# dfdazac/grapes

Measured on AMD Instinct MI355X. Metric: sampled edges aggregated/sec, ogbn-products 3-layer GFlowNet, higher is better.
Workload: dtype f32

## Files before the change

grapes_amd/_lib.py:

```python
from __future__ import annotations

import ctypes as C
import os

_HERE = os.path.dirname(os.path.abspath(__file__))
DIAG_LIB_PATH = os.path.join(_HERE, "libgrapes_hip_diag.so")
DIAG = os.environ.get("GRAPES_DIAG", "0") == "1"
LIB_PATH = os.environ.get("GRAPES_LIB_PATH") or (DIAG_LIB_PATH if DIAG else os.path.join(_HERE, "libgrapes_hip.so"))
ABI_MAJOR, ABI_MINOR = 3, 2


def diag_switch(name: str, default: str) -> str:
    if os.environ.get("GRAPES_DIAG", "0") == "1":
        return os.environ.get(name, default)
    return default


P = C.c_void_p
I32 = C.c_int32
I64 = C.c_int64
U32 = C.c_uint32
U64 = C.c_uint64
F32 = C.c_float
SZ = C.c_size_t
# ... 135 lines not shown
    "grapes_sampler_head_bwd_multi_phase": (I32, [I32, P, P, P, P, P, P, P, P, P, P, P, P, I32, P, P, P, I32, P]),
    "grapes_linear_bias_act_head_fwd_strided": (I32, [P, I32, P, P, I32, P, P, P, I32, P, I32, I32, P]),
    "grapes_linear_bwd_weight_gated_strided": (I32, [P, P, I32, P, I32, P, P, P, P, P, I32, I32, I32, P, P]),
    "grapes_linear_bwd_weight_gated_workspace_bytes": (SZ, [I32, I32, I32]),
    "grapes_linear_bwd_weight_gated": (I32, [P, P, P, P, P, I32, P, I32, I32, I32, P, P, P, P, P]),
    "grapes_linear_bwd_weight_gated_multi": (I32, [I32, P, P, P, P, P, P, P, P, P, I32, I32, I32, P, P]),
    "grapes_linear_bwd_weight_slabs_bytes": (SZ, [I32, I32, I32]),
    "grapes_linear_bwd_weight_slabs": (I32, [P, P, P, I32, P, I32, I32, I32, P, P]),
    "grapes_linear_bwd_weight_slabs_and_input": (I32, [P, P, P, P, P, I32, P, I32, I32, I32, P, P]),
    "grapes_slab_reduce_sets": (I32, [I32, P, P, P, I32, P, I32, P]),
    "grapes_gcn_aggregate_narrow_pair": (I32, [P, P, P, P, P, P, P, P, P, I32, P, P]),
    "grapes_linear_relu_head_fwd_bits": (I32, [P, I32, P, P, P, P, P, I32, P, I32, I32, P]),
    "grapes_linear_relu_head_fwd_bits_pair": (I32, [P, I32, P, P, P, P, P, P, I32, P, P, P, P, P, I32, I32, P, I32, I32, P]),
    "grapes_linear_bwd_weight_bits_multi_cols": (I32, [I32, P, P, P, P, P, P, P, P, P, P, I32, P, P, I32, I32, I32, P, P]),
    "grapes_linear_bwd_weight_bits_pair_cols": (I32, [I32, P, P, P, P, P, P, P, P, P, P, I32, P, P, I32, P, P, P, P, P, P, I32, I32, I32, P, P]),
    "grapes_gcn_aggregate_gather_fwd": (I32, [P, I32, I32, P, P, U32, P, I32, P, P, P, P, P, I32, P, P]),
    "grapes_gcn_aggregate_gather_fwd_peers": (I32, [P, P, I32, I32, I32, P, P, U32, P, I32, P, P, P, P, P, I32, P, P]),
    "grapes_peer_export": (I32, [P, P, P]),
    "grapes_peer_open": (I32, [P, U64, P]),
    "grapes_peer_close": (I32, [P, U64]),
    "grapes_peer_copy": (I32, [P, P, SZ, P]),
    "grapes_gcn_aggregate_workspace_bytes": (SZ, [I32, I32]),
    "grapes_gcn_aggregate_fwd": (I32, [P, P, P, P, P, P, I32, P, I32, I32, P, P, I32, P, P]),
    "grapes_gcn_aggregate_fwd_head": (I32, [P, P, P, P, P, P, I32, P, I32, I32, P, P, P, P]),
    "grapes_gcn_aggregate_fwd_prescaled": (I32, [P, P, P, P, P, P, I32, P, I32, I32, P, P, I32, P, P]),
    "grapes_scale_rows": (I32, [P, P, P, I64, I32, P]),
    "grapes_gcn_aggregate_bwd_rank1_workspace_bytes": (SZ, [I32, I32]),
    "grapes_gcn_aggregate_bwd_rank1": (I32, [P, P, P, P, P, P, P, P, P, I32, I32, P, I32, P, P, I32, P, P]),
    "grapes_gcn_aggregate_bwd_rank1_bits": (I32, [P, P, P, P, P, P, P, P, P, P, I32, I32, P, I32, P, P, I32, P, P]),
    "grapes_gcn_aggregate_bwd_rank1_bits_multi": (I32, [I32, P, P, P, P, P, P, P, P, P, P, P, P, P, I32, P, P, P, P, P]),
# ... 104 lines not shown
```

grapes_amd/csrc/gemm_kernels.hip:

```cpp
#include <type_traits>
#include "common.h"
#include <cstdlib>

typedef float f32x16 __attribute__((ext_vector_type(16)));

#define GB_M 128
#define GB_N 128
#define GB_K 16
#define GB_LD 132

struct GatherOp { const int32_t* ids; const uint32_t* code; const uint32_t* d_epoch; uint32_t epoch; int F; uint32_t mask; };

template <bool KMAJOR, bool VEC>
__device__ __forceinline__ void gemm_load_tile(const float* __restrict__ P, long long ld, int r0, int R, int k0,
                                               int kend, int tid, float4 (&v)[2], const float* __restrict__ G = nullptr,
                                               int ones_at = -1, const float* __restrict__ row_scale = nullptr,
                                               const float* __restrict__ col_vec = nullptr, float4* cs2 = nullptr,
                                               const GatherOp* go = nullptr, bool do_cs2 = false) {
    if (VEC) {
#pragma unroll
        for (int i = 0; i < 2; ++i) {
            int k, r;
            bool ok;
            long long off;
// ... 1805 lines not shown
}

#define DS_NT 128
#ifdef GRAPES_STAMPS
#define DWS_STAMP(slot, T0) do { if (grapes_stamp_ptr && threadIdx.x == (T0) && blockIdx.x < 64) grapes_stamp_ptr[blockIdx.x * 16 + (slot)] = wall_clock64(); } while (0)
#define DWS_STAMP_IT(it_, slot) do { if ((it_) == 6) { DWS_STAMP(slot, 0); DWS_STAMP((slot) + 6, 256); } } while (0)
#else
#define DWS_STAMP(slot, T0) do { } while (0)
#define DWS_STAMP_IT(it_, slot) do { } while (0)
#endif
#define DS_MINROWS 128
__host__ __device__ __forceinline__ int dw_share(int total, int nwg, bool min_rows) {
    const int per = (total + nwg - 1) / nwg;
    return (min_rows && per < DS_MINROWS) ? DS_MINROWS : per;
}
struct DwAlt { int nwg0; int first_seg; int Nin; const float* cv; float* slabs; float* cs_db; };
struct DwsRegs { uint32_t gw[8]; float4 xb[4]; float rsb[4]; float rso; int rows; float4 xb2[4]; float rsb2[4]; float rso2; };
struct DwsCtx { int M, Nin, kb, ac4, bshift, hb, bc4, ok_, hb2, bc42, ok2_, lane; bool a_role, b_role, o_role, b2_role, o2_role; };
__device__ __forceinline__ int dws_sw(int n) { return n ^ ((n >> 3) & 3); }
template <int ROLE, int NT, int G>
__device__ __forceinline__ void dws_stage_slice(const DwsRegs& R, const DwsCtx& c, uint4* __restrict__ WA, char* __restrict__ WB,
                                                uint4* __restrict__ dummy) {
    constexpr int B_PL = 4 * NT;
    char* dm = reinterpret_cast<char*>(&dummy[c.lane]);
    if constexpr (G < 4) {
        constexpr int u = G;
        if constexpr (ROLE == 0) {
            uint32_t e[4];
#pragma unroll
            for (int pq = 0; pq < 4; ++pq) {
                const uint32_t n0 = (8 * c.kb + 2 * pq < R.rows) ? (R.gw[2 * pq] >> c.bshift) & 15u : 0u;
// ... 56 lines not shown
}
template <int ROLE, int NT>
__device__ __forceinline__ void dws_stage_set(const DwsRegs& R, const DwsCtx& c, uint4* __restrict__ WA, char* __restrict__ WB,
                                              uint4* __restrict__ dummy) {
    dws_stage_slice<ROLE, NT, 0>(R, c, WA, WB, dummy);
    dws_stage_slice<ROLE, NT, 1>(R, c, WA, WB, dummy);
    dws_stage_slice<ROLE, NT, 2>(R, c, WA, WB, dummy);
    dws_stage_slice<ROLE, NT, 3>(R, c, WA, WB, dummy);
    dws_stage_slice<ROLE, NT, 4>(R, c, WA, WB, dummy);
}
template <bool BITS, int NT = 128>
__global__ __launch_bounds__(512, 1) void gemm_dw_split_k(DwSegs sg, const float* __restrict__ cv_, int M, int Nin_,
                                                          float* __restrict__ slabs_, float* __restrict__ cs_db_,
                                                          float* __restrict__ cs_head, DwAlt alt) {
    extern __shared__ uint4 ds_smem[];
    const bool dual = alt.nwg0 < (int)gridDim.x, p1 = dual && (int)blockIdx.x >= alt.nwg0;
    const int bid = p1 ? (int)blockIdx.x - alt.nwg0 : (int)blockIdx.x;
    const int nwg = p1 ? (int)gridDim.x - alt.nwg0 : (dual ? alt.nwg0 : (int)gridDim.x);
    const int seg_lo = p1 ? alt.first_seg : 0, seg_hi = (dual && !p1) ? alt.first_seg : sg.nseg;
    const int Nin = p1 ? alt.Nin : Nin_;
    const float* __restrict__ cv = p1 ? alt.cv : cv_;
    float* __restrict__ slabs = p1 ? alt.slabs : slabs_;
    float* __restrict__ cs_db = p1 ? alt.cs_db : cs_db_;
    auto sw = [](int n) { return n ^ ((n >> 3) & 3); };
    constexpr int A_IMG = 4 * DW_MAXM, B_PL = 4 * NT, BUF = A_IMG + 3 * B_PL;
    constexpr int TN = NT / 32;
    const int tid = threadIdx.x, lane = tid & 63, wid = tid >> 6;
    const int li = lane & 31, h = lane >> 5;
    DWS_STAMP(0, 0);
    for (int i = tid; i < 2 * BUF; i += 512) ds_smem[i] = make_uint4(0u, 0u, 0u, 0u);
    int nrows[4], off[5];
    off[0] = 0;
    {
// ... 343 lines not shown
    if (BITS) {
    } else if (cs_head) {
        __syncthreads();
        float* red = reinterpret_cast<float*>(ds_smem);
        if (a_role) *reinterpret_cast<float4*>(&red[kb * M + 4 * ac4]) = cs2;
        __syncthreads();
        if (tid < M) cs_head[(long long)bid * M + tid] = ((red[tid] + red[M + tid]) + red[2 * M + tid]) + red[3 * M + tid];
    }
}
#define SR1_G 8
struct Sr1Prob {
    const float* slabs; const float* tslabs; const float* cv; const float* W1; const float* b1;
    float* dw; float* db; float* dwh; int nwg, Nin, seg_lo, seg_hi;
    int dw_cols;
};
template <int NC, int G>
__global__ __launch_bounds__(NC * G) void slab_reduce_rank1_k(DwSegs sg, Sr1Prob pa, Sr1Prob pb, int M, int accumulate) {
    __shared__ float red[NC / 64];
    const Sr1Prob P = blockIdx.y ? pb : pa;
    const int Nin = P.Nin;
    const int m = blockIdx.x, g = threadIdx.x / NC, n = threadIdx.x - g * NC;
    const bool is_s = n < Nin, is_t = n == Nin;
    int cnt[4];
#pragma unroll
    for (int q = 0; q < 4; ++q) {
        const bool has = q < sg.nseg && sg.d_n[q];
        const int32_t raw = *(has ? sg.d_n[q] : reinterpret_cast<const int32_t*>(P.cv));
        cnt[q] = has ? raw : 0x7fffffff;
    }
    const float c = P.cv[m];
    const float wrow = (g == 0 && P.dwh) ? (is_s ? P.W1[(long long)m * Nin + n] : (is_t ? P.b1[m] : 0.f)) : 0.f;
    float* o = is_s ? (n < P.dw_cols ? P.dw + (long long)m * P.dw_cols + n : nullptr) : ((is_t && P.db) ? P.db + m : nullptr);
    const float prev = (g == 0 && accumulate && o) ? *o : 0.f;
    int total = 0;
#pragma unroll
    for (int q = 0; q < 4; ++q)
        total += (q >= P.seg_lo && q < P.seg_hi) ? (cnt[q] < sg.n_cap[q] ? (cnt[q] > 0 ? cnt[q] : 0) : sg.n_cap[q]) : 0;
    const int per = dw_share(total, P.nwg, true);
    const int live = total > 0 ? (total + per - 1) / per : 0;
    constexpr int Q = NC / 4, NG = NC * G / Q;
    __shared__ float part4[NG][NC];
    const int q4 = threadIdx.x % Q, g4 = threadIdx.x / Q;
    const bool q_s = 4 * q4 < Nin, q_t = 4 * q4 == Nin;
    float4 a4 = make_float4(0.f, 0.f, 0.f, 0.f);
    if (q_s || q_t) {
// ... 5 lines not shown
                const int z = zb + u * NG < live ? zb + u * NG : live - 1;
                v[u] = q_t ? make_float4(P.tslabs[(long long)z * M + m], 0.f, 0.f, 0.f)
                           : *reinterpret_cast<const float4*>(base + (long long)z * Nin);
            }
#pragma unroll
            for (int u = 0; u < 8; ++u)
                if (zb + u * NG < live) { a4.x += v[u].x; a4.y += v[u].y; a4.z += v[u].z; a4.w += v[u].w; }
        }
    }
    if (4 * q4 + 3 < NC) *reinterpret_cast<float4*>(&part4[g4][4 * q4]) = a4;
    __syncthreads();
    if (g == 0) {
        float sum = part4[0][n];
#pragma unroll 8
        for (int q = 1; q < NG; ++q) sum += part4[q][n];
        if (o) *o = prev + c * sum;
        if (P.dwh) {
            const float p = wave_sum(sum * wrow);
            if ((n & 63) == 0) red[n >> 6] = p;
        }
    }
    __syncthreads();
    if (P.dwh && threadIdx.x == 0) {
        float t = red[0] + red[1];
        if (NC > 128) t += red[2];
        P.dwh[m] = accumulate ? P.dwh[m] + t : t;
    }
}

#define DS_NT_WIDE 160
static inline bool dw_split_ok(int f_in, int f_out, bool bits = false) {
    const bool shape = f_out % 32 == 0 && f_out >= 32 && f_out <= DW_MAXM && f_in % 4 == 0 && f_in >= 4;
    if (shape && 8 * (f_in / 4) + DW_KC <= 256) return true;
    return bits && shape && f_in + 1 <= DS_NT_WIDE && 8 * (f_in / 4) + DW_KC <= 256 + 64;
}
static inline bool dw_split_narrow(int f_in) { return 8 * (f_in / 4) + DW_KC <= 256; }

static inline bool dw_rank1_ok(int f_in, int f_out) {
    return f_out % 32 == 0 && f_out >= 32 && f_out <= DW_MAXM && f_in % 4 == 0 && f_in >= 4 && f_in + 1 <= DW_NT &&
           (512 % (f_out / 4)) == 0;
}

static inline bool fused_dw_ok(const float* dout, const float* gate, const float* x, int f_in, int f_out) {
    return grapes_aligned16(dout) && grapes_aligned16(x) && (!gate || grapes_aligned16(gate)) && f_in % 4 == 0 && f_out % 4 == 0 &&
           f_in % GB_N != 0;
}

#define DW_BLOCKS 256
#define DW_BLOCKS_SECOND 32
struct DwSecond { const float* col_vec; const float* w1; const float* b1; float* dw; float* dbias; float* dw_head; int f_in; };
static int launch_dw_rank1(int nseg, const float* const* gate, const float* const* x, const float* const* row_scale,
                           const int32_t* const* d_n, const int32_t* n_cap, const float* col_vec, float* dw, float* dbias,
                           float* dw_head, int f_in, int f_out, int accumulate, void* workspace, hipStream_t s,
                           const int32_t* x_stride = nullptr ,
                           const uint32_t* const* bits = nullptr ,
                           const float* w1 = nullptr, const float* b1 = nullptr,
                           const struct DwSecond* second = nullptr ,
                           int dw_cols = 0 ) {
    static bool attr_set = false;
    const size_t lds = (size_t)(2 * DW_KC * DW_LDA + 2 * DW_KC * DW_LDB) * sizeof(float);
    if (!attr_set) {
        hipError_t e = hipFuncSetAttribute((const void*)gemm_dw_rank1_k, hipFuncAttributeMaxDynamicSharedMemorySize, (int)lds);
        if (e != hipSuccess) return (int)e;
        attr_set = true;
    }
    DwSegs sg;
    sg.nseg = nseg;
    for (int h = 0; h < 4; ++h) {
        const int q = h < nseg ? h : 0;
        sg.gate[h] = gate ? gate[q] : nullptr; sg.x[h] = x[q]; sg.rs[h] = row_scale[q]; sg.d_n[h] = d_n[q]; sg.n_cap[h] = h < nseg ? n_cap[q] : 0;
        sg.ldx[h] = (x_stride && x_stride[q] > 0) ? x_stride[q] : f_in;
        sg.bits[h] = bits ? bits[q] : nullptr;
    }
// ... 20 lines not shown
            hipError_t e = hipFuncSetAttribute((const void*)gemm_dw_split_k<false>, hipFuncAttributeMaxDynamicSharedMemorySize, (int)l128);
            if (e != hipSuccess) return (int)e;
            e = hipFuncSetAttribute((const void*)gemm_dw_split_k<true>, hipFuncAttributeMaxDynamicSharedMemorySize, (int)l128);
            if (e != hipSuccess) return (int)e;
            e = hipFuncSetAttribute((const void*)gemm_dw_split_k<true, DS_NT_WIDE>, hipFuncAttributeMaxDynamicSharedMemorySize, (int)l160);
            if (e != hipSuccess) return (int)e;
            attr2_set = true;
        }
        if (bits) {
            static int second_wgs = -1;
            if (second_wgs < 0) { const char* e = grapes_tune_env("GRAPES_DW_SECOND_WGS"); second_wgs = e ? atoi(e) : DW_BLOCKS_SECOND;
                                  if (second_wgs < 8 || second_wgs > 128) second_wgs = DW_BLOCKS_SECOND; }
            const int nwg0 = second ? DW_BLOCKS - second_wgs : DW_BLOCKS;
            float* w_dw2 = w_dw + (size_t)nwg0 * slab;
            float* w_db2 = w_db + (size_t)nwg0 * f_out;
            const DwAlt alt{nwg0, second ? nseg - 1 : nseg, second ? second->f_in : f_in, second ? second->col_vec : col_vec, w_dw2, w_db2};
            if (wide)
                hipLaunchKernelGGL((gemm_dw_split_k<true, DS_NT_WIDE>), dim3(DW_BLOCKS), dim3(512), lds2, s, sg, col_vec, f_out, f_in, w_dw, w_db,
                                   (float*)nullptr, alt);
            else
                hipLaunchKernelGGL(gemm_dw_split_k<true>, dim3(DW_BLOCKS), dim3(512), lds2, s, sg, col_vec, f_out, f_in, w_dw, w_db,
                                   (float*)nullptr, alt);
            GRAPES_LAUNCH_CHECK();
            const Sr1Prob pa{w_dw, w_db, col_vec, w1, b1, dw, dbias, dw_head, nwg0, f_in, 0, second ? nseg - 1 : nseg,
                             dw_cols > 0 ? dw_cols : f_in};
            const Sr1Prob pb = second ? Sr1Prob{w_dw2, w_db2, second->col_vec, second->w1, second->b1, second->dw, second->dbias,
                                                second->dw_head, DW_BLOCKS - nwg0, second->f_in, nseg - 1, nseg, second->f_in} : pa;
            if (wide)
                hipLaunchKernelGGL((slab_reduce_rank1_k<192, 5>), dim3(f_out, second ? 2 : 1), dim3(192 * 5), 0, s, sg, pa, pb, f_out, accumulate);
            else
                hipLaunchKernelGGL((slab_reduce_rank1_k<128, SR1_G>), dim3(f_out, second ? 2 : 1), dim3(128 * SR1_G), 0, s, sg, pa, pb, f_out, accumulate);
            GRAPES_LAUNCH_CHECK();
            return 0;
        }
        const DwAlt none{DW_BLOCKS, nseg, f_in, col_vec, w_dw, w_db};
        hipLaunchKernelGGL(gemm_dw_split_k<false>, dim3(DW_BLOCKS), dim3(512), lds2, s, sg, col_vec, f_out, f_in, w_dw,
                           dbias ? w_db : nullptr, dw_head ? w_dh : nullptr, none);
    } else {
        hipLaunchKernelGGL(gemm_dw_rank1_k, dim3(DW_BLOCKS), dim3(512), lds, s, sg, col_vec, f_out, f_in, w_dw,
                           dbias ? w_db : nullptr, dw_head ? w_dh : nullptr);
    }
    GRAPES_LAUNCH_CHECK();
    int grid = grapes_div_up(slab, 64); if (grid > 4096) grid = 4096;
    const int g2 = grid + (dbias ? grapes_div_up(f_out, 64) : 0) + (dw_head ? grapes_div_up(f_out, 64) : 0);
    hipLaunchKernelGGL(slab_reduce_k, dim3(g2), dim3(256), 0, s, (const float*)w_dw, dw, slab, DW_BLOCKS, (const int32_t*)nullptr, 1,
                       accumulate, (const float*)(dbias ? w_db : nullptr), dbias, (long long)(dbias ? f_out : 0),
                       (const float*)(dw_head ? w_dh : nullptr), dw_head, (long long)(dw_head ? f_out : 0));
    GRAPES_LAUNCH_CHECK();
    return 0;
}
// ... 265 lines not shown
    if (dw_cols < 0 || dw_cols > f_in || (dw_cols > 0 && f_in - dw_cols > 3)) return GRAPES_EINVAL;
    if (dw_head && (!w1 || !b1)) return GRAPES_EINVAL;
    int nmax = 0;
    for (int h = 0; h < nseg; ++h) {
        if (!gate_bits[h] || !x[h] || !row_scale[h] || n_cap[h] <= 0) return GRAPES_EINVAL;
        if (x_stride && x_stride[h] > 0 && (x_stride[h] < f_in || (x_stride[h] & 3))) return GRAPES_EINVAL;
        if (!grapes_aligned16(x[h])) return GRAPES_EALIGN;
        nmax = n_cap[h] > nmax ? n_cap[h] : nmax;
    }
    if (!grapes_aligned16(col_vec)) return GRAPES_EALIGN;
    if (!grapes_split_gemm_available(nmax > 2048 ? nmax : 2048, f_in, f_out)) return GRAPES_EINVAL;
    if (dw_cols > 0 && dw_cols != f_in && !dw_split_ok(f_in, f_out, true)) return GRAPES_EINVAL;
    return launch_dw_rank1(nseg, nullptr, x, row_scale, d_n, n_cap, col_vec, dw, dbias, dw_head, f_in, f_out, accumulate, workspace,
                           (hipStream_t)stream, x_stride, gate_bits, w1, b1, nullptr, dw_cols);
}
extern "C" int grapes_linear_bwd_weight_bits_pair_cols(int32_t nseg, const uint32_t* const* gate_bits, const float* const* x,
                                                       const int32_t* x_stride, const float* const* row_scale,
                                                       const int32_t* const* d_n, const int32_t* n_cap, const float* col_vec,
                                                       const float* w1, const float* b1, float* dw, int32_t dw_cols, float* dbias,
                                                       float* dw_head, int32_t f_in, const float* col_vec_b, const float* w1_b,
                                                       const float* b1_b, float* dw_b, float* dbias_b, float* dw_head_b,
                                                       int32_t f_in_b, int32_t f_out, int32_t accumulate, void* workspace,
                                                       grapes_stream_t stream) {
    if (nseg < 1 || nseg > 3 || !gate_bits || !x || !row_scale || !d_n || !n_cap || !col_vec || !dw || !workspace) return GRAPES_EINVAL;
    if (dw_cols < 0 || dw_cols > f_in || (dw_cols > 0 && f_in - dw_cols > 3)) return GRAPES_EINVAL;
    if (!col_vec_b || !dw_b || f_in_b <= 0 || f_in_b > f_in) return GRAPES_EINVAL;
    if ((dw_head && (!w1 || !b1)) || (dw_head_b && (!w1_b || !b1_b))) return GRAPES_EINVAL;
    int nmax = 0;
    for (int h = 0; h <= nseg; ++h) {
        const int fi = h < nseg ? f_in : f_in_b;
        if (!gate_bits[h] || !x[h] || !row_scale[h] || n_cap[h] <= 0) return GRAPES_EINVAL;
        if (x_stride && x_stride[h] > 0 && (x_stride[h] < fi || (x_stride[h] & 3))) return GRAPES_EINVAL;
        if (!grapes_aligned16(x[h])) return GRAPES_EALIGN;
        nmax = n_cap[h] > nmax ? n_cap[h] : nmax;
    }
    if (!grapes_aligned16(col_vec) || !grapes_aligned16(col_vec_b)) return GRAPES_EALIGN;
    if (!grapes_split_gemm_available(nmax > 2048 ? nmax : 2048, f_in, f_out) ||
        !grapes_split_gemm_available(nmax > 2048 ? nmax : 2048, f_in_b, f_out)) return GRAPES_EINVAL;
    int32_t strides[4];
    for (int h = 0; h <= nseg; ++h) strides[h] = (x_stride && x_stride[h] > 0) ? x_stride[h] : (h < nseg ? f_in : f_in_b);
    const DwSecond sec{col_vec_b, w1_b, b1_b, dw_b, dbias_b, dw_head_b, f_in_b};
    return launch_dw_rank1(nseg + 1, nullptr, x, row_scale, d_n, n_cap, col_vec, dw, dbias, dw_head, f_in, f_out, accumulate, workspace,
                           (hipStream_t)stream, strides, gate_bits, w1, b1, &sec, dw_cols);
}
```

grapes_amd/ops.py:

```python
from __future__ import annotations

from typing import List, Optional

import ctypes as _C
import os

import torch

from . import _lib
from ._lib import diag_switch as _sw

_i32 = torch.int32
_i64 = torch.int64
_f32 = torch.float32


def lib():
    return _lib.load()


def _stream() -> int:
    try:
        return torch._C._cuda_getCurrentRawStream(torch._C._cuda_getDevice())
    except AttributeError:
# ... 823 lines not shown
        raise ValueError("linear_bwd_weight_bits_multi: w1 must be a dense [f_out, f_in] matrix and b1 [f_out]")
    dw_cols = _dw_cols(dw, fo, fi, "linear_bwd_weight_bits_multi")
    strides = (C.c_int32 * nseg)(*[_row_strided(x, fi, "linear_bwd_weight_bits_multi") for x in xs])
    arr = lambda ts: (C.c_void_p * nseg)(*[t.data_ptr() for t in ts])
    caps = (C.c_int32 * nseg)(*[x.shape[0] for x in xs])
    ws = _ws(lib().grapes_linear_bwd_weight_gated_workspace_bytes(1, fi, fo), dw.device)
    _lib.check(lib().grapes_linear_bwd_weight_bits_multi_cols(nseg, arr([b.words for b in bits]), arr(xs), strides, arr(row_scales),
                                                              arr(d_ns), caps, _p(col_vec), _p(w1), _p(b1), _p(dw), dw_cols,
                                                              _p(dbias), _p(dw_head), fi, fo, 1 if accumulate else 0, _p(ws),
                                                              _stream()),
               "linear_bwd_weight_bits_multi")
    return dw


def linear_bwd_weight_bits_pair(bits, xs, row_scales, d_ns, col_vec, w1, b1, dw, dbias, dw_head,
                                bits_b, x_b, row_scale_b, d_n_b, col_vec_b, w1_b, b1_b, dw_b, dbias_b, dw_head_b, accumulate=False):
    import ctypes as C
    nseg = len(bits)
    if not (1 <= nseg <= 3 and len(xs) == nseg and len(row_scales) == nseg and len(d_ns) == nseg):
        raise ValueError("1..3 row sets of layer a with matching operand lists")
    for t in list(row_scales) + [row_scale_b, col_vec, col_vec_b, dw, dw_b, w1, b1, w1_b, b1_b]:
        _chk(t, _f32, "operand")
    fo, fi, fib = bits[0].f_out, xs[0].shape[1], x_b.shape[1]
    if (bits_b.f_out != fo or tuple(w1.shape) != (fo, fi) or tuple(w1_b.shape) != (fo, fib) or not w1.is_contiguous() or
            not w1_b.is_contiguous()):
        raise ValueError("linear_bwd_weight_bits_pair: dense [f_out, f_in] weights of one f_out")
    allx = list(xs) + [x_b]
    strides = (C.c_int32 * (nseg + 1))(*[_row_strided(x, fi if i < nseg else fib, "linear_bwd_weight_bits_pair") for i, x in enumerate(allx)])
    arr = lambda ts: (C.c_void_p * (nseg + 1))(*[t.data_ptr() for t in ts])
    caps = (C.c_int32 * (nseg + 1))(*[x.shape[0] for x in allx])
    ws = _ws(lib().grapes_linear_bwd_weight_gated_workspace_bytes(1, fi, fo), dw.device)
    dw_cols = _dw_cols(dw, fo, fi, "linear_bwd_weight_bits_pair")
    _lib.check(lib().grapes_linear_bwd_weight_bits_pair_cols(
        nseg, arr([b.words for b in bits] + [bits_b.words]), arr(allx), strides, arr(list(row_scales) + [row_scale_b]),
        arr(list(d_ns) + [d_n_b]), caps, _p(col_vec), _p(w1), _p(b1), _p(dw), dw_cols, _p(dbias), _p(dw_head), fi,
        _p(col_vec_b), _p(w1_b), _p(b1_b), _p(dw_b), _p(dbias_b), _p(dw_head_b), fib, fo, 1 if accumulate else 0, _p(ws),
        _stream()), "linear_bwd_weight_bits_pair")
    return dw, dw_b


def pad_features(X):
    F = X.shape[1]
    if F % 4 == 0:
        return X.contiguous(), F
    Xp = torch.zeros((X.shape[0], (F + 3) // 4 * 4), dtype=X.dtype, device=X.device)
    Xp[:, :F] = X
    return Xp, F


class FeaturePlanes:

    def __init__(self, Xp: torch.Tensor):
        _chk(Xp, _f32, "X")
# ... 1527 lines not shown
```

grapes_amd/step_graph.py:

```python
from __future__ import annotations

import contextlib
import copy
from typing import Dict, List, Optional

import os

import torch

from ._lib import diag_switch as _sw
import torch.nn as nn

from . import ops
from .capture import SegmentedGraph
from .graph import DeviceGraph


class _FirstLayer:

    def __init__(self, conv, F, num_ind, legacy=False):
        self.conv, self.F, self.num_ind = conv, F, num_ind
        self.K = F + num_ind
        self.Kp = self.K if legacy else (self.K + 3) // 4 * 4
        self.agg_first = legacy or self.K < conv.out_channels or conv.out_channels % 4 != 0
# ... 789 lines not shown
            main_s.wait_stream(self._side)
        elif not cb_done:
            self._classifier_backward(s)

    def _nets_backward(self, s, carry_bwd) -> bool:
        hops, num_ind, ep = self.hops, self.num_ind, self.epoch_t
        gf1, gf2, st_gf, z1, z2, st_z = self._nets()
        hop_state, zstate, gscale = s.hop_state, s.zstate, s.gscale
        z_done = False
        cb_done = False
        fi_, fo_ = st_gf.Kp, gf1.out_channels
        multi = hops <= 4 and st_gf.agg_first and fi_ % 4 == 0 and fi_ % 128 != 0 and fo_ % 4 == 0
        heads = multi or (hops <= 4 and all(hs.get("cand_pos") is not None for hs in hop_state) and
                          _sw("GRAPES_HEAD_BWD_MULTI", "1") != "0")
        dh2s, z_dh2 = None, None
        if heads:
            z_rides = (not self.reinforce) and hops <= 3
            zs = [zstate] if z_rides else []
            hb = ops.SamplerHeadBwdMulti([hs["logit"].view(-1) for hs in hop_state] + [z["zout"].view(-1) for z in zs],
                                         [hs["mask"] for hs in hop_state] + [None for _ in zs],
                                         [hs["cand_pos"] for hs in hop_state] + [None for _ in zs],
                                         [hs["prep"] for hs in hop_state] + [z["prep"] for z in zs],
                                         d_grad_scale=gscale, sum_out=gf2.bias.grad, accumulate_sum=False,
                                         mean_sum_out=z2.bias.grad if z_rides else None)
            if carry_bwd:
                if self._rider_end_hook is not None:
                    self._rider_end_hook()
                ops.carry_backward_aggregations([lambda: hb.launch(1), lambda: hb.launch(2)])
                try:
                    self._classifier_backward(s)
                finally:
                    ops.flush_backward_hosts()
                cb_done = True
            else:
                hb.launch(0)
            dh2_all = hb.dh
            dh2s = [dh2_all[h][:hs["logit"].numel()] for h, hs in enumerate(hop_state)]
            z_dh2 = dh2_all[hops][:zstate["zout"].numel()].view(-1, 1) if z_rides else None
        if multi:
            if all(isinstance(hs["act1"], ops.GateBits) for hs in hop_state):
                if (z_dh2 is not None and isinstance(zstate["act"], ops.GateBits) and hops <= 3 and
                        zstate["x"].shape[1] <= st_gf.Kp and _sw("GRAPES_DW_PAIR", "1") != "0"):
                    ops.linear_bwd_weight_bits_pair(
                        [hs["act1"] for hs in hop_state], [hs["x"] for hs in hop_state], dh2s, [hs["prep"].d_n for hs in hop_state],
                        gf2.lin.weight.view(-1), st_gf.weight, gf1.bias, st_gf.grad_direct, gf1.bias.grad, gf2.lin.weight.grad.view(-1),
                        zstate["act"], zstate["x"], z_dh2.view(-1), zstate["prep"].d_n, z2.lin.weight.view(-1), st_z.weight, z1.bias,
                        st_z.grad, z1.bias.grad, z2.lin.weight.grad.view(-1), accumulate=False)
                    z_done = True
                else:
                    ops.linear_bwd_weight_bits_multi([hs["act1"] for hs in hop_state], [hs["x"] for hs in hop_state], dh2s,
                                                     [hs["prep"].d_n for hs in hop_state], gf2.lin.weight.view(-1), st_gf.weight,
                                                     gf1.bias, st_gf.grad_direct, dbias=gf1.bias.grad,
                                                     dw_head=gf2.lin.weight.grad.view(-1), accumulate=False)
            else:
                ops.linear_bwd_weight_gated_multi([hs["act1"] for hs in hop_state], [hs["x"] for hs in hop_state], dh2s,
                                                  [hs["prep"].d_n for hs in hop_state], gf2.lin.weight.view(-1),
                                                  st_gf.grad, dbias=gf1.bias.grad,
                                                  dw_head=gf2.lin.weight.grad.view(-1), accumulate=False)
        dh_r1s, z_r1 = [None] * len(hop_state), None
        if (dh2s is not None and not multi and _sw("GRAPES_R1_MULTI", "1") != "0" and
                all(self._r1_ok(gf1, hs["act1"]) for hs in hop_state)):
            z_in = (z_dh2 is not None and not (self.reinforce or z_done) and self._r1_ok(z1, zstate["act"]) and
# ... 376 lines not shown
```

include/grapes_hip.h:

```cpp
#ifndef GRAPES_HIP_H
#define GRAPES_HIP_H

#include <stddef.h>
#include <stdint.h>

#ifdef __cplusplus
extern "C" {
#endif

#define GRAPES_ABI_VERSION 302

#define GRAPES_EINVAL (-1)
#define GRAPES_EALIGN (-2)

#define GRAPES_STATUS_EDGE_OVERFLOW 1
#define GRAPES_STATUS_NODE_OVERFLOW 2
#define GRAPES_STATUS_BAD_INDEX 4
#define GRAPES_STATUS_SYNC_TIMEOUT 8
#define GRAPES_SYNC_WORDS 256

typedef void* grapes_stream_t;

int grapes_abi_version(void);
const char* grapes_target_arch(void);
// ... 193 lines not shown
                                          const float* head_w_b, uint32_t* gate_bits_b, float* head_out_b, int32_t f_in_b,
                                          int32_t n, const int32_t* d_n, int32_t f_in, int32_t f_out, grapes_stream_t stream);
int grapes_linear_bwd_weight_bits_multi_cols(int32_t nseg, const uint32_t* const* gate_bits, const float* const* x,
                                             const int32_t* x_stride, const float* const* row_scale,
                                             const int32_t* const* d_n, const int32_t* n_cap, const float* col_vec,
                                             const float* w1, const float* b1, float* dw, int32_t dw_cols, float* dbias,
                                             float* dw_head, int32_t f_in, int32_t f_out, int32_t accumulate, void* workspace,
                                             grapes_stream_t stream);
int grapes_linear_bwd_weight_bits_pair_cols(int32_t nseg, const uint32_t* const* gate_bits, const float* const* x,
                                            const int32_t* x_stride, const float* const* row_scale,
                                            const int32_t* const* d_n, const int32_t* n_cap, const float* col_vec,
                                            const float* w1, const float* b1, float* dw, int32_t dw_cols, float* dbias,
                                            float* dw_head, int32_t f_in, const float* col_vec_b, const float* w1_b,
                                            const float* b1_b, float* dw_b, float* dbias_b, float* dw_head_b, int32_t f_in_b,
                                            int32_t f_out, int32_t accumulate, void* workspace, grapes_stream_t stream);
size_t grapes_linear_bwd_weight_gated_workspace_bytes(int32_t n_cap, int32_t f_in, int32_t f_out);
int grapes_linear_bwd_weight_gated(const float* dout, const float* gate, const float* x, float* dw,
                                   float* dbias, int32_t n, const int32_t* d_n, int32_t f_in,
                                   int32_t f_out, int32_t accumulate, const float* row_scale,
                                   const float* col_vec, float* dw_head, void* workspace, grapes_stream_t stream);
int grapes_linear_bwd_weight_gated_multi(int32_t nseg, const float* const* gate, const float* const* x,
                                         const float* const* row_scale, const int32_t* const* d_n,
                                         const int32_t* n_cap, const float* col_vec, float* dw, float* dbias,
                                         float* dw_head, int32_t f_in, int32_t f_out, int32_t accumulate,
                                         void* workspace, grapes_stream_t stream);
#ifdef GRAPES_DIAG
int grapes_debug_gemm_fwd(const float* x, const float* w, float* out, int32_t n, int32_t f_in,
                          int32_t f_out, int32_t dbg, grapes_stream_t stream);
int grapes_debug_gather_probe(const float* X, int32_t x_stride, const int32_t* row_head, float* out, int32_t n,
                              int32_t f_out, int32_t variant, int32_t grid_cap, grapes_stream_t stream);
// ... 409 lines not shown
```

Before: 505.0 million.

## Defer gradient-scale multiply into dW slab reduction and allow split workgroup launches

The sampler head backward now runs without the device-side gradient scale, and the scale is applied once later in the rank-1 slab reduce kernel. That kernel multiplies dW, dbias and dw_head by delta, using an fma error term, and rescales the two bias-grad scalars. The dW split-K kernel also gains a workgroup range (wg_lo/wg_hi) and a reduce flag, so it can be launched in pieces, although the default call launches all shares at once. This moves the per-element scaling out of the earlier stage, at the cost of extra parameters and an ordering dependency on the scalar rescale.

```diff
diff --git a/grapes_amd/_lib.py b/grapes_amd/_lib.py
--- a/grapes_amd/_lib.py
+++ b/grapes_amd/_lib.py
@@ -173,6 +173,9 @@
     "grapes_linear_relu_head_fwd_bits_pair": (I32, [P, I32, P, P, P, P, P, P, I32, P, P, P, P, P, I32, I32, P, I32, I32, P]),
     "grapes_linear_bwd_weight_bits_multi_cols": (I32, [I32, P, P, P, P, P, P, P, P, P, P, I32, P, P, I32, I32, I32, P, P]),
     "grapes_linear_bwd_weight_bits_pair_cols": (I32, [I32, P, P, P, P, P, P, P, P, P, P, I32, P, P, I32, P, P, P, P, P, P, I32, I32, I32, P, P]),
+    "grapes_linear_bwd_weight_shares": (I32, []),
+    "grapes_linear_bwd_weight_bits_pair_unscaled": (I32, [I32, P, P, P, P, P, P, P, P, P, P, I32, P, P, I32, P, P, P, P, P, P, I32, I32, I32, P,
+                                                          I32, I32, I32, P, P, P, P]),
     "grapes_gcn_aggregate_gather_fwd": (I32, [P, I32, I32, P, P, U32, P, I32, P, P, P, P, P, I32, P, P]),
     "grapes_gcn_aggregate_gather_fwd_peers": (I32, [P, P, I32, I32, I32, P, P, U32, P, I32, P, P, P, P, P, I32, P, P]),
     "grapes_peer_export": (I32, [P, P, P]),
diff --git a/grapes_amd/csrc/gemm_kernels.hip b/grapes_amd/csrc/gemm_kernels.hip
--- a/grapes_amd/csrc/gemm_kernels.hip
+++ b/grapes_amd/csrc/gemm_kernels.hip
@@ -1843,7 +1843,7 @@
     const int per = (total + nwg - 1) / nwg;
     return (min_rows && per < DS_MINROWS) ? DS_MINROWS : per;
 }
-struct DwAlt { int nwg0; int first_seg; int Nin; const float* cv; float* slabs; float* cs_db; };
+struct DwAlt { int nwg0; int first_seg; int Nin; const float* cv; float* slabs; float* cs_db; int wg_lo; int wg_total; };
 struct DwsRegs { uint32_t gw[8]; float4 xb[4]; float rsb[4]; float rso; int rows; float4 xb2[4]; float rsb2[4]; float rso2; };
 struct DwsCtx { int M, Nin, kb, ac4, bshift, hb, bc4, ok_, hb2, bc42, ok2_, lane; bool a_role, b_role, o_role, b2_role, o2_role; };
 __device__ __forceinline__ int dws_sw(int n) { return n ^ ((n >> 3) & 3); }
@@ -1930,9 +1930,10 @@
                                                           float* __restrict__ slabs_, float* __restrict__ cs_db_,
                                                           float* __restrict__ cs_head, DwAlt alt) {
     extern __shared__ uint4 ds_smem[];
-    const bool dual = alt.nwg0 < (int)gridDim.x, p1 = dual && (int)blockIdx.x >= alt.nwg0;
-    const int bid = p1 ? (int)blockIdx.x - alt.nwg0 : (int)blockIdx.x;
-    const int nwg = p1 ? (int)gridDim.x - alt.nwg0 : (dual ? alt.nwg0 : (int)gridDim.x);
+    const int wg = (int)blockIdx.x + alt.wg_lo;
+    const bool dual = alt.nwg0 < alt.wg_total, p1 = dual && wg >= alt.nwg0;
+    const int bid = p1 ? wg - alt.nwg0 : wg;
+    const int nwg = p1 ? alt.wg_total - alt.nwg0 : (dual ? alt.nwg0 : alt.wg_total);
     const int seg_lo = p1 ? alt.first_seg : 0, seg_hi = (dual && !p1) ? alt.first_seg : sg.nseg;
     const int Nin = p1 ? alt.Nin : Nin_;
     const float* __restrict__ cv = p1 ? alt.cv : cv_;
@@ -2306,8 +2307,9 @@
     float* dw; float* db; float* dwh; int nwg, Nin, seg_lo, seg_hi;
     int dw_cols;
 };
+struct Sr1Delta { const float* d_delta; float* scalar[2]; };
 template <int NC, int G>
-__global__ __launch_bounds__(NC * G) void slab_reduce_rank1_k(DwSegs sg, Sr1Prob pa, Sr1Prob pb, int M, int accumulate) {
+__global__ __launch_bounds__(NC * G) void slab_reduce_rank1_k(DwSegs sg, Sr1Prob pa, Sr1Prob pb, int M, int accumulate, Sr1Delta dl) {
     __shared__ float red[NC / 64];
     const Sr1Prob P = blockIdx.y ? pb : pa;
     const int Nin = P.Nin;
@@ -2320,7 +2322,8 @@
         const int32_t raw = *(has ? sg.d_n[q] : reinterpret_cast<const int32_t*>(P.cv));
         cnt[q] = has ? raw : 0x7fffffff;
     }
-    const float c = P.cv[m];
+    const float delta = dl.d_delta ? *dl.d_delta : 1.f;
+    const float c = P.cv[m], cd = c * delta, ce = fmaf(c, delta, -cd);
     const float wrow = (g == 0 && P.dwh) ? (is_s ? P.W1[(long long)m * Nin + n] : (is_t ? P.b1[m] : 0.f)) : 0.f;
     float* o = is_s ? (n < P.dw_cols ? P.dw + (long long)m * P.dw_cols + n : nullptr) : ((is_t && P.db) ? P.db + m : nullptr);
     const float prev = (g == 0 && accumulate && o) ? *o : 0.f;
@@ -2356,7 +2359,7 @@
         float sum = part4[0][n];
 #pragma unroll 8
         for (int q = 1; q < NG; ++q) sum += part4[q][n];
-        if (o) *o = prev + c * sum;
+        if (o) *o = dl.d_delta ? fmaf(cd, sum, fmaf(ce, sum, prev)) : prev + c * sum;
         if (P.dwh) {
             const float p = wave_sum(sum * wrow);
             if ((n & 63) == 0) red[n >> 6] = p;
@@ -2366,7 +2369,12 @@
     if (P.dwh && threadIdx.x == 0) {
         float t = red[0] + red[1];
         if (NC > 128) t += red[2];
+        if (dl.d_delta) t *= delta;
         P.dwh[m] = accumulate ? P.dwh[m] + t : t;
+    }
+    if (dl.d_delta && threadIdx.x == 0 && blockIdx.x == 0 && blockIdx.y == 0) {
+        if (dl.scalar[0]) *dl.scalar[0] *= delta;
+        if (dl.scalar[1]) *dl.scalar[1] *= delta;
     }
 }
 
@@ -2390,6 +2398,7 @@
 
 #define DW_BLOCKS 256
 #define DW_BLOCKS_SECOND 32
+struct DwPhase { int wg_lo, wg_hi, reduce; const float* d_delta; float* scalar[2]; };
 struct DwSecond { const float* col_vec; const float* w1; const float* b1; float* dw; float* dbias; float* dw_head; int f_in; };
 static int launch_dw_rank1(int nseg, const float* const* gate, const float* const* x, const float* const* row_scale,
                            const int32_t* const* d_n, const int32_t* n_cap, const float* col_vec, float* dw, float* dbias,
@@ -2398,7 +2407,8 @@
                            const uint32_t* const* bits = nullptr ,
                            const float* w1 = nullptr, const float* b1 = nullptr,
                            const struct DwSecond* second = nullptr ,
-                           int dw_cols = 0 ) {
+                           int dw_cols = 0 ,
+                           const struct DwPhase* ph = nullptr ) {
     static bool attr_set = false;
     const size_t lds = (size_t)(2 * DW_KC * DW_LDA + 2 * DW_KC * DW_LDB) * sizeof(float);
     if (!attr_set) {
@@ -2449,26 +2459,33 @@
             const int nwg0 = second ? DW_BLOCKS - second_wgs : DW_BLOCKS;
             float* w_dw2 = w_dw + (size_t)nwg0 * slab;
             float* w_db2 = w_db + (size_t)nwg0 * f_out;
-            const DwAlt alt{nwg0, second ? nseg - 1 : nseg, second ? second->f_in : f_in, second ? second->col_vec : col_vec, w_dw2, w_db2};
-            if (wide)
-                hipLaunchKernelGGL((gemm_dw_split_k<true, DS_NT_WIDE>), dim3(DW_BLOCKS), dim3(512), lds2, s, sg, col_vec, f_out, f_in, w_dw, w_db,
-                                   (float*)nullptr, alt);
-            else
-                hipLaunchKernelGGL(gemm_dw_split_k<true>, dim3(DW_BLOCKS), dim3(512), lds2, s, sg, col_vec, f_out, f_in, w_dw, w_db,
-                                   (float*)nullptr, alt);
-            GRAPES_LAUNCH_CHECK();
+            const int wg_lo = ph ? ph->wg_lo : 0, wg_hi = ph ? ph->wg_hi : DW_BLOCKS;
+            if (wg_lo < 0 || wg_hi > DW_BLOCKS) return GRAPES_EINVAL;
+            const DwAlt alt{nwg0, second ? nseg - 1 : nseg, second ? second->f_in : f_in, second ? second->col_vec : col_vec, w_dw2, w_db2,
+                            wg_lo, DW_BLOCKS};
+            if (wg_hi > wg_lo) {
+                if (wide)
+                    hipLaunchKernelGGL((gemm_dw_split_k<true, DS_NT_WIDE>), dim3(wg_hi - wg_lo), dim3(512), lds2, s, sg, col_vec, f_out, f_in, w_dw, w_db,
+                                       (float*)nullptr, alt);
+                else
+                    hipLaunchKernelGGL(gemm_dw_split_k<true>, dim3(wg_hi - wg_lo), dim3(512), lds2, s, sg, col_vec, f_out, f_in, w_dw, w_db,
+                                       (float*)nullptr, alt);
+                GRAPES_LAUNCH_CHECK();
+            }
+            if (ph && !ph->reduce) return 0;
+            const Sr1Delta dl{ph ? ph->d_delta : nullptr, {ph ? ph->scalar[0] : nullptr, ph ? ph->scalar[1] : nullptr}};
             const Sr1Prob pa{w_dw, w_db, col_vec, w1, b1, dw, dbias, dw_head, nwg0, f_in, 0, second ? nseg - 1 : nseg,
                              dw_cols > 0 ? dw_cols : f_in};
             const Sr1Prob pb = second ? Sr1Prob{w_dw2, w_db2, second->col_vec, second->w1, second->b1, second->dw, second->dbias,
                                                 second->dw_head, DW_BLOCKS - nwg0, second->f_in, nseg - 1, nseg, second->f_in} : pa;
             if (wide)
-                hipLaunchKernelGGL((slab_reduce_rank1_k<192, 5>), dim3(f_out, second ? 2 : 1), dim3(192 * 5), 0, s, sg, pa, pb, f_out, accumulate);
+                hipLaunchKernelGGL((slab_reduce_rank1_k<192, 5>), dim3(f_out, second ? 2 : 1), dim3(192 * 5), 0, s, sg, pa, pb, f_out, accumulate, dl);
             else
-                hipLaunchKernelGGL((slab_reduce_rank1_k<128, SR1_G>), dim3(f_out, second ? 2 : 1), dim3(128 * SR1_G), 0, s, sg, pa, pb, f_out, accumulate);
+                hipLaunchKernelGGL((slab_reduce_rank1_k<128, SR1_G>), dim3(f_out, second ? 2 : 1), dim3(128 * SR1_G), 0, s, sg, pa, pb, f_out, accumulate, dl);
             GRAPES_LAUNCH_CHECK();
             return 0;
         }
-        const DwAlt none{DW_BLOCKS, nseg, f_in, col_vec, w_dw, w_db};
+        const DwAlt none{DW_BLOCKS, nseg, f_in, col_vec, w_dw, w_db, 0, DW_BLOCKS};
         hipLaunchKernelGGL(gemm_dw_split_k<false>, dim3(DW_BLOCKS), dim3(512), lds2, s, sg, col_vec, f_out, f_in, w_dw,
                            dbias ? w_db : nullptr, dw_head ? w_dh : nullptr, none);
     } else {
@@ -2764,14 +2781,14 @@
     return launch_dw_rank1(nseg, nullptr, x, row_scale, d_n, n_cap, col_vec, dw, dbias, dw_head, f_in, f_out, accumulate, workspace,
                            (hipStream_t)stream, x_stride, gate_bits, w1, b1, nullptr, dw_cols);
 }
-extern "C" int grapes_linear_bwd_weight_bits_pair_cols(int32_t nseg, const uint32_t* const* gate_bits, const float* const* x,
+static int bits_pair_impl(int32_t nseg, const uint32_t* const* gate_bits, const float* const* x,
                                                        const int32_t* x_stride, const float* const* row_scale,
                                                        const int32_t* const* d_n, const int32_t* n_cap, const float* col_vec,
                                                        const float* w1, const float* b1, float* dw, int32_t dw_cols, float* dbias,
                                                        float* dw_head, int32_t f_in, const float* col_vec_b, const float* w1_b,
                                                        const float* b1_b, float* dw_b, float* dbias_b, float* dw_head_b,
                                                        int32_t f_in_b, int32_t f_out, int32_t accumulate, void* workspace,
-                                                       grapes_stream_t stream) {
+                                                       grapes_stream_t stream, const DwPhase* ph) {
     if (nseg < 1 || nseg > 3 || !gate_bits || !x || !row_scale || !d_n || !n_cap || !col_vec || !dw || !workspace) return GRAPES_EINVAL;
     if (dw_cols < 0 || dw_cols > f_in || (dw_cols > 0 && f_in - dw_cols > 3)) return GRAPES_EINVAL;
     if (!col_vec_b || !dw_b || f_in_b <= 0 || f_in_b > f_in) return GRAPES_EINVAL;
@@ -2791,5 +2808,31 @@
     for (int h = 0; h <= nseg; ++h) strides[h] = (x_stride && x_stride[h] > 0) ? x_stride[h] : (h < nseg ? f_in : f_in_b);
     const DwSecond sec{col_vec_b, w1_b, b1_b, dw_b, dbias_b, dw_head_b, f_in_b};
     return launch_dw_rank1(nseg + 1, nullptr, x, row_scale, d_n, n_cap, col_vec, dw, dbias, dw_head, f_in, f_out, accumulate, workspace,
-                           (hipStream_t)stream, strides, gate_bits, w1, b1, &sec, dw_cols);
-}
+                           (hipStream_t)stream, strides, gate_bits, w1, b1, &sec, dw_cols, ph);
+}
+extern "C" int grapes_linear_bwd_weight_bits_pair_cols(int32_t nseg, const uint32_t* const* gate_bits, const float* const* x,
+                                                       const int32_t* x_stride, const float* const* row_scale,
+                                                       const int32_t* const* d_n, const int32_t* n_cap, const float* col_vec,
+                                                       const float* w1, const float* b1, float* dw, int32_t dw_cols, float* dbias,
+                                                       float* dw_head, int32_t f_in, const float* col_vec_b, const float* w1_b,
+                                                       const float* b1_b, float* dw_b, float* dbias_b, float* dw_head_b,
+                                                       int32_t f_in_b, int32_t f_out, int32_t accumulate, void* workspace,
+                                                       grapes_stream_t stream) {
+    return bits_pair_impl(nseg, gate_bits, x, x_stride, row_scale, d_n, n_cap, col_vec, w1, b1, dw, dw_cols, dbias, dw_head, f_in,
+                          col_vec_b, w1_b, b1_b, dw_b, dbias_b, dw_head_b, f_in_b, f_out, accumulate, workspace, stream, nullptr);
+}
+extern "C" int32_t grapes_linear_bwd_weight_shares(void) { return DW_BLOCKS; }
+extern "C" int grapes_linear_bwd_weight_bits_pair_unscaled(int32_t nseg, const uint32_t* const* gate_bits, const float* const* x,
+                                                           const int32_t* x_stride, const float* const* row_scale,
+                                                           const int32_t* const* d_n, const int32_t* n_cap, const float* col_vec,
+                                                           const float* w1, const float* b1, float* dw, int32_t dw_cols, float* dbias,
+                                                           float* dw_head, int32_t f_in, const float* col_vec_b, const float* w1_b,
+                                                           const float* b1_b, float* dw_b, float* dbias_b, float* dw_head_b,
+                                                           int32_t f_in_b, int32_t f_out, int32_t accumulate, void* workspace,
+                                                           int32_t wg_lo, int32_t wg_hi, int32_t reduce, const float* d_delta,
+                                                           float* scalar_a, float* scalar_b, grapes_stream_t stream) {
+    if (wg_lo < 0 || wg_hi > DW_BLOCKS || wg_hi < wg_lo || (wg_hi == wg_lo && !reduce)) return GRAPES_EINVAL;
+    const DwPhase ph{wg_lo, wg_hi, reduce, d_delta, {scalar_a, scalar_b}};
+    return bits_pair_impl(nseg, gate_bits, x, x_stride, row_scale, d_n, n_cap, col_vec, w1, b1, dw, dw_cols, dbias, dw_head, f_in,
+                          col_vec_b, w1_b, b1_b, dw_b, dbias_b, dw_head_b, f_in_b, f_out, accumulate, workspace, stream, &ph);
+}
diff --git a/grapes_amd/ops.py b/grapes_amd/ops.py
--- a/grapes_amd/ops.py
+++ b/grapes_amd/ops.py
@@ -861,7 +861,8 @@
 
 
 def linear_bwd_weight_bits_pair(bits, xs, row_scales, d_ns, col_vec, w1, b1, dw, dbias, dw_head,
-                                bits_b, x_b, row_scale_b, d_n_b, col_vec_b, w1_b, b1_b, dw_b, dbias_b, dw_head_b, accumulate=False):
+                                bits_b, x_b, row_scale_b, d_n_b, col_vec_b, w1_b, b1_b, dw_b, dbias_b, dw_head_b, accumulate=False,
+                                unscaled=None):
     import ctypes as C
     nseg = len(bits)
     if not (1 <= nseg <= 3 and len(xs) == nseg and len(row_scales) == nseg and len(d_ns) == nseg):
@@ -876,14 +877,33 @@
     strides = (C.c_int32 * (nseg + 1))(*[_row_strided(x, fi if i < nseg else fib, "linear_bwd_weight_bits_pair") for i, x in enumerate(allx)])
     arr = lambda ts: (C.c_void_p * (nseg + 1))(*[t.data_ptr() for t in ts])
     caps = (C.c_int32 * (nseg + 1))(*[x.shape[0] for x in allx])
-    ws = _ws(lib().grapes_linear_bwd_weight_gated_workspace_bytes(1, fi, fo), dw.device)
+    u = unscaled
+    ws = u.get("ws") if u else None
+    if ws is None:
+        ws = dw_pair_workspace(fi, fo, dw.device)
     dw_cols = _dw_cols(dw, fo, fi, "linear_bwd_weight_bits_pair")
-    _lib.check(lib().grapes_linear_bwd_weight_bits_pair_cols(
-        nseg, arr([b.words for b in bits] + [bits_b.words]), arr(allx), strides, arr(list(row_scales) + [row_scale_b]),
-        arr(list(d_ns) + [d_n_b]), caps, _p(col_vec), _p(w1), _p(b1), _p(dw), dw_cols, _p(dbias), _p(dw_head), fi,
-        _p(col_vec_b), _p(w1_b), _p(b1_b), _p(dw_b), _p(dbias_b), _p(dw_head_b), fib, fo, 1 if accumulate else 0, _p(ws),
-        _stream()), "linear_bwd_weight_bits_pair")
+    args = (nseg, arr([b.words for b in bits] + [bits_b.words]), arr(allx), strides, arr(list(row_scales) + [row_scale_b]),
+            arr(list(d_ns) + [d_n_b]), caps, _p(col_vec), _p(w1), _p(b1), _p(dw), dw_cols, _p(dbias), _p(dw_head), fi,
+            _p(col_vec_b), _p(w1_b), _p(b1_b), _p(dw_b), _p(dbias_b), _p(dw_head_b), fib, fo, 1 if accumulate else 0, _p(ws))
+    if u is None:
+        _lib.check(lib().grapes_linear_bwd_weight_bits_pair_cols(*args, _stream()), "linear_bwd_weight_bits_pair")
+        return dw, dw_b
+    scal = list(u.get("scalars") or ()) + [None, None]
+    for t in scal[:2] + [u.get("delta")]:
+        _chk(t, _f32, "unscaled operand", True)
+    lo, hi = u.get("shares") or (0, dw_shares())
+    _lib.check(lib().grapes_linear_bwd_weight_bits_pair_unscaled(
+        *args, int(lo), int(hi), 1 if u.get("reduce", True) else 0, _p(u.get("delta")), _p(scal[0]), _p(scal[1]), _stream()),
+        "linear_bwd_weight_bits_pair_unscaled")
     return dw, dw_b
+
+
+def dw_shares() -> int:
+    return int(lib().grapes_linear_bwd_weight_shares())
+
+
+def dw_pair_workspace(f_in, f_out, device):
+    return _ws(lib().grapes_linear_bwd_weight_gated_workspace_bytes(1, f_in, f_out), device)
 
 
 def pad_features(X):
diff --git a/grapes_amd/step_graph.py b/grapes_amd/step_graph.py
--- a/grapes_amd/step_graph.py
+++ b/grapes_amd/step_graph.py
@@ -827,14 +827,18 @@
         heads = multi or (hops <= 4 and all(hs.get("cand_pos") is not None for hs in hop_state) and
                           _sw("GRAPES_HEAD_BWD_MULTI", "1") != "0")
         dh2s, z_dh2 = None, None
+        unscaled = False
         if heads:
             z_rides = (not self.reinforce) and hops <= 3
             zs = [zstate] if z_rides else []
+            unscaled = (multi and z_rides and all(isinstance(hs["act1"], ops.GateBits) for hs in hop_state) and
+                        isinstance(zstate["act"], ops.GateBits) and zstate["x"].shape[1] <= st_gf.Kp and
+                        _sw("GRAPES_DW_PAIR", "1") != "0" and _sw("GRAPES_BWD_UNSCALED", "1") != "0")
             hb = ops.SamplerHeadBwdMulti([hs["logit"].view(-1) for hs in hop_state] + [z["zout"].view(-1) for z in zs],
                                          [hs["mask"] for hs in hop_state] + [None for _ in zs],
                                          [hs["cand_pos"] for hs in hop_state] + [None for _ in zs],
                                          [hs["prep"] for hs in hop_state] + [z["prep"] for z in zs],
-                                         d_grad_scale=gscale, sum_out=gf2.bias.grad, accumulate_sum=False,
+                                         d_grad_scale=None if unscaled else gscale, sum_out=gf2.bias.grad, accumulate_sum=False,
                                          mean_sum_out=z2.bias.grad if z_rides else None)
             if carry_bwd:
                 if self._rider_end_hook is not None:
@@ -858,7 +862,8 @@
                         [hs["act1"] for hs in hop_state], [hs["x"] for hs in hop_state], dh2s, [hs["prep"].d_n for hs in hop_state],
                         gf2.lin.weight.view(-1), st_gf.weight, gf1.bias, st_gf.grad_direct, gf1.bias.grad, gf2.lin.weight.grad.view(-1),
                         zstate["act"], zstate["x"], z_dh2.view(-1), zstate["prep"].d_n, z2.lin.weight.view(-1), st_z.weight, z1.bias,
-                        st_z.grad, z1.bias.grad, z2.lin.weight.grad.view(-1), accumulate=False)
+                        st_z.grad, z1.bias.grad, z2.lin.weight.grad.view(-1), accumulate=False,
+                        unscaled=dict(delta=gscale, scalars=(gf2.bias.grad, z2.bias.grad)) if unscaled else None)
                     z_done = True
                 else:
                     ops.linear_bwd_weight_bits_multi([hs["act1"] for hs in hop_state], [hs["x"] for hs in hop_state], dh2s,
diff --git a/include/grapes_hip.h b/include/grapes_hip.h
--- a/include/grapes_hip.h
+++ b/include/grapes_hip.h
@@ -231,6 +231,16 @@
                                             float* dw_head, int32_t f_in, const float* col_vec_b, const float* w1_b,
                                             const float* b1_b, float* dw_b, float* dbias_b, float* dw_head_b, int32_t f_in_b,
                                             int32_t f_out, int32_t accumulate, void* workspace, grapes_stream_t stream);
+int32_t grapes_linear_bwd_weight_shares(void);
+int grapes_linear_bwd_weight_bits_pair_unscaled(int32_t nseg, const uint32_t* const* gate_bits, const float* const* x,
+                                                const int32_t* x_stride, const float* const* row_scale,
+                                                const int32_t* const* d_n, const int32_t* n_cap, const float* col_vec,
+                                                const float* w1, const float* b1, float* dw, int32_t dw_cols, float* dbias,
+                                                float* dw_head, int32_t f_in, const float* col_vec_b, const float* w1_b,
+                                                const float* b1_b, float* dw_b, float* dbias_b, float* dw_head_b, int32_t f_in_b,
+                                                int32_t f_out, int32_t accumulate, void* workspace, int32_t wg_lo, int32_t wg_hi,
+                                                int32_t reduce, const float* d_delta, float* scalar_a, float* scalar_b,
+                                                grapes_stream_t stream);
 size_t grapes_linear_bwd_weight_gated_workspace_bytes(int32_t n_cap, int32_t f_in, int32_t f_out);
 int grapes_linear_bwd_weight_gated(const float* dout, const float* gate, const float* x, float* dw,
                                    float* dbias, int32_t n, const int32_t* d_n, int32_t f_in,
```

After: 501.9 million. No clear change (-0.6%).
